# colopl/libpoporon

Hardware: AMD Instinct MI355X
Metric: RS(255,223) codewords/s (encode; decode @ t=16 errs) and GB/s vs HBM peak, 1/2/4/8 GPU (higher is better)
Workload: dtype u8; 1 GPU; RS(255,223) round trip: encode + decode with 16 errors per codeword, 1048576 codewords per GPU (BASELINE configs[1]+[2]); codewords_per_gpu=1048576, layout=255-byte codeword rows, stride 255, code=poporon_config_rs_default (8, 0x11D, fcr 1, prim 1, 32 roots)

## Files before the change

__graft_entry__.py:

```python
import os
import subprocess
import sys
import time

ROOT = os.path.dirname(os.path.abspath(__file__))


def build() -> None:
    subprocess.check_call(["make", "-j8", "-C", os.path.join(ROOT, "libpoporon_amd")])
    subprocess.check_call(["make", "-C", os.path.join(ROOT, "testutil")])
    subprocess.check_call(["make", "-C", os.path.join(ROOT, "tests", "c")])
    subprocess.check_call(["make", "-C", os.path.join(ROOT, "oracle")])
    if ROOT not in sys.path:
        sys.path.insert(0, ROOT)
    import libpoporon_amd

    libpoporon_amd.load_library()


def _errors(rng, bad, span, nerr, exclude=None):
    import numpy as np
    n = bad.shape[0]
    key = rng.random((n, span))
    if exclude is not None:
        np.put_along_axis(key, exclude.astype(np.int64), -1.0, axis=1)
    nmax = int(np.max(nerr))
    pos = np.argsort(-key, axis=1)[:, :nmax]
    mag = rng.integers(1, 256, (n, nmax), dtype=np.uint8)
    if not np.isscalar(nerr):
        mag[np.arange(nmax)[None, :] >= np.asarray(nerr)[:, None]] = 0
    r = np.arange(n)[:, None]
    bad[r, pos] ^= mag
    return pos


def smoke() -> None:
    if ROOT not in sys.path:
        sys.path.insert(0, ROOT)
    import numpy as np
    import torch

    import libpoporon_amd as P
    from oracle import Oracle

    assert torch.cuda.is_available(), "smoke() needs cuda:0"
    torch.cuda.set_device(0)
    t0 = time.perf_counter()
    prev_path = os.environ.get("POPORON_AMD_DECODE_PATH")
    os.environ["POPORON_AMD_DECODE_PATH"] = "split"
    try:
        rs = P.Poporon.default(device=0)
    finally:
        if prev_path is None:
            del os.environ["POPORON_AMD_DECODE_PATH"]
        else:
            os.environ["POPORON_AMD_DECODE_PATH"] = prev_path
    o = Oracle()
    th = min(16, os.cpu_count() or 1)
    rng = np.random.default_rng(0x5EED0001)
    n = 1 << 16
    K, NR = 223, 32
    s = torch.cuda.current_stream().cuda_stream

    data = rng.integers(0, 256, (n, K), dtype=np.uint8)
    cw = torch.zeros((n, 255), dtype=torch.uint8, device="cuda")
    cw[:, :K] = torch.from_numpy(data).cuda()
    rs.encode_batch_device(cw.data_ptr(), 255, cw.data_ptr() + K, 255, K, n, s)
    torch.cuda.synchronize()
    enc = cw.cpu().numpy()
    assert (enc[:, K:] == o.encode_batch(data, threads=th)).all(), "encode parity mismatch vs oracle"
    print(f"smoke encode: {n} messages, parity bit-exact vs oracle (rs_lfsr_k<ENCODE>)", flush=True)

    names = P.KERNEL_NAMES

    def decode(label, bad, expect, slots=None, cnt=None, kernels=""):
        d = torch.from_numpy(bad).cuda()
        ok = torch.zeros(n, dtype=torch.uint8, device="cuda")
        cor = torch.zeros(n, dtype=torch.uint8, device="cuda")
        kw = {}
        if slots is not None:
            sd = torch.from_numpy(np.ascontiguousarray(slots)).cuda()
            cd = torch.from_numpy(np.ascontiguousarray(cnt)).cuda()
            kw = dict(d_positions=sd.data_ptr(), positions_stride=slots.shape[1], d_counts=cd.data_ptr())
        rs.timing(True)
        rs.decode_batch_device(d.data_ptr(), 255, d.data_ptr() + K, 255, K, n, ok.data_ptr(), cor.data_ptr(),
                               stream=s, **kw)
        torch.cuda.synchronize()
        t = {k: rs.timing_read(k) for k in names}
        rs.timing(False)
        ran = {k for k, (ms, c) in t.items() if c}
        missing = [names[k] for k in expect if k not in ran]
        assert not missing, f"{label}: kernels that did not run: {missing}"
        assert P.KERNEL_CORRECT not in ran, f"{label}: the whole-batch general kernel ran instead of the split path"
        if slots is None:
            want = o.decode_batch(bad[:, :K], bad[:, K:], threads=th)
        else:
            want = o.decode_batch(bad[:, :K], bad[:, K:], slots.astype(np.uint32), cnt.astype(np.uint32), threads=th)
        out = d.cpu().numpy()
        gok, gcor = ok.cpu().numpy(), cor.cpu().numpy()
        assert (gok == want[0]).all(), f"{label}: ok differs at {np.nonzero(gok != want[0])[0][:8]}"
        assert (gcor == want[1]).all(), f"{label}: corrected_num differs at {np.nonzero(gcor != want[1])[0][:8]}"
        diff = np.nonzero((out[:, :K] != want[2]).any(1) | (out[:, K:] != want[3]).any(1))[0]
        assert diff.size == 0, f"{label}: decoded bytes differ at codewords {diff[:8]}"
        print(f"smoke {label}: {n} codewords bit-exact vs oracle (bytes, ok, corrected_num); ok {int(gok.sum())}, "
              f"corrected {int(gcor.sum())}; ran {kernels or ', '.join(names[k] for k in sorted(ran))}", flush=True)
        return gok, gcor, out

    bad = enc.copy()
    _errors(rng, bad, 255, 16)
    gok, gcor, out = decode("decode16", bad, (P.KERNEL_REMAINDER, P.KERNEL_BM, P.KERNEL_CHIEN, P.KERNEL_FORNEY,
                                              P.KERNEL_APPLY, P.KERNEL_LIST),
                            kernels="rs_lfsr_k<SYNDROME>, rs_bm_k, rs_chien_k, rs_forney_k, rs_apply_k<16>, "
                                    "rs_wave_k (list, empty)")
    assert gok.all() and (gcor == 16).all() and (out == enc).all()

    bad = enc.copy()
    slots = np.sort(np.argsort(rng.random((n, K)), axis=1)[:, :NR], axis=1).astype(np.uint8)
    bad[np.arange(n)[:, None], slots] ^= rng.integers(1, 256, (n, NR), dtype=np.uint8)
    cnt = np.full(n, NR, np.uint8)
    gok, gcor, out = decode("erasure32", bad, (P.KERNEL_REMAINDER, P.KERNEL_ERASURE, P.KERNEL_APPLY), slots, cnt,
                            kernels="rs_lfsr_k<SYNDROME>, rs_era_bp_k, rs_apply_k<32>")
    assert gok.all() and (gcor == NR).all() and (out == enc).all()

    bad = enc.copy()
    era = np.argsort(rng.random((n, K)), axis=1)[:, :16]
    slots = rng.integers(0, 255, (n, NR)).astype(np.uint8)
    slots[:, :16] = era
    bad[np.arange(n)[:, None], era] ^= rng.integers(1, 256, (n, 16), dtype=np.uint8)
    _errors(rng, bad, 255, 8, exclude=era)
    cnt = np.full(n, 16, np.uint8)
    decode("errata16e8", bad, (P.KERNEL_REMAINDER, P.KERNEL_ERASURE, P.KERNEL_BM, P.KERNEL_CHIEN, P.KERNEL_FORNEY,
                               P.KERNEL_APPLY, P.KERNEL_LIST), slots, cnt,
           kernels="rs_lfsr_k<SYNDROME>, rs_era_bp_k (hand-off), rs_ebm_k, rs_chien32_k, rs_forney32_k, "
                   "rs_wave_k (list), rs_apply_k<32>")

    bad = enc.copy()
    ne = np.minimum(rng.binomial(255, 0.045, n), 24)
    _errors(rng, bad, 255, ne)
    gok, _, _ = decode("mixed", bad, (P.KERNEL_REMAINDER, P.KERNEL_BM, P.KERNEL_CHIEN, P.KERNEL_FORNEY,
                                      P.KERNEL_APPLY, P.KERNEL_LIST),
                       kernels="rs_lfsr_k<SYNDROME>, rs_bm_k, rs_chien_k, rs_forney_k, rs_apply_k<16>, "
                               "rs_wave_k (list: L > 16 / deg != L, one wave per codeword)")
    assert (ne > 16).sum() > n // 50 and (gok == 0).sum() > 0

    for c in range(8):
        par = rs.encode(data[c])
        assert (par == enc[c, K:]).all(), "poporon_encode mismatch"
        b = enc[c].copy()
        _errors(rng, b[None, :], 255, 16 + (c & 1) * 2)
        got = rs.decode(b[:K], b[K:])
        want = o.decode(b[:K], b[K:])
        assert got[0] == want[0] and got[1] == want[1] and (got[2] == want[2]).all() and (got[3] == want[3]).all()
    print("smoke single calls: 8 x poporon_encode + poporon_decode (16 / 18 errors) bit-exact vs oracle "
          "(the single-call server rs_serve_k: enc1_body / dec1_body)", flush=True)
    print(f"smoke ok ({time.perf_counter() - t0:.1f} s)", flush=True)


if __name__ == "__main__":
    build()
    if len(sys.argv) > 1 and sys.argv[1] == "smoke":
        smoke()
```

libpoporon_amd/csrc/api.cpp:

```cpp
#include <hip/hip_runtime.h>

#include <algorithm>
#include <atomic>
#include <chrono>
#include <cstdarg>
#include <cstdio>
#include <cstdlib>
#include <cstring>
#include <mutex>
#include <new>
#include <string>
#include <thread>
#include <vector>

#include "poporon.h"
#include "poporon_amd.h"
#include "rs_device.h"
#include "rs_generic.h"
#include "bch_device.h"

#ifndef POPORON_BUILDTIME
#define POPORON_BUILDTIME 1
#endif
#define POPORON_VERSION_ID 20000000
// ... 68 lines not shown

struct GpuCtx {
    bool timing = false;
    std::vector<TimedLaunch> pending;
    std::vector<hipEvent_t> event_pool;
    double total_ms[NKERN] = {};
    uint64_t launches[NKERN] = {};
    bool ready = false;
    int device = -1;
    int num_cu = 256;
    hipStream_t stream = nullptr;
    RsDevTables *tab = nullptr;
    RsGenTables *gtab = nullptr;
    uint8_t *rem = nullptr;
    size_t rem_cap = 0;
    hipEvent_t rem_done = nullptr;
    hipStream_t rem_stream = nullptr;
    bool rem_pending = false;
    uint8_t *stage = nullptr;
    uint8_t *hstage = nullptr;
    uint8_t *zc = nullptr, *zc_dev = nullptr;
    uint32_t zc_seq = 0;
    hipStream_t sstream = nullptr;
    bool srv_on = false;
    uint32_t srv_id = 0;
    uint32_t srv_seq = 0;
    size_t stage_cap = 0;
    bool registered = false;
    bool batch_open = false;
    bool batch_ev_live = false;
    hipEvent_t batch_ev = nullptr;
    struct PipeSlot {
        hipStream_t stream = nullptr;
        hipEvent_t done = nullptr;
        uint8_t *host = nullptr;
        uint8_t *dev = nullptr;
        size_t cap = 0;
        bool busy = false;
        size_t c0 = 0, n = 0;
    } pipe[3];
};
#define PIPE_SLOTS 3

struct _poporon_t {
    poporon_fec_type_t fec_type;
    poporon_rs_t *rs;
    uint16_t primitive_inverse;
    poporon_erasure_t *erasure;
    uint16_t *ext_syndrome;
    size_t last_corrected;
    bool supported;
    bool fast;
    int decode_path;
    bool generic;
    bool lfsr_nr;
    bool nrsplit;
    int gen_path;
    RsDevTables host_tab;
    RsCorrParams corr;
    RsGenTables gen_tab;
    RsGenParams gen;
    poporon_gf_t *bgf;
    BchParams bch;
    bool bch_ok;
    GpuCtx gpu;
};


static inline uint8_t gf_mod(const poporon_gf_t *gf, uint16_t v)
{
    while (v >= gf->field_size) {
        v = (uint16_t)(v - gf->field_size);
        v = (uint16_t)((v >> gf->symbol_size) + (v & gf->field_size));
    }
    return (uint8_t)v;
}

EXPORT void poporon_gf_destroy(poporon_gf_t *gf)
{
    if (!gf)
        return;
    free(gf->log2exp);
    free(gf->exp2log);
    free(gf);
}

EXPORT poporon_gf_t *poporon_gf_create(uint8_t symbol_size, uint16_t generator_polynomial)
{
    if (symbol_size < 1 || symbol_size > 16)
        return nullptr;
    poporon_gf_t *gf = (poporon_gf_t *)calloc(1, sizeof(poporon_gf_t));
    if (!gf)
        return nullptr;
    gf->symbol_size = symbol_size;
    gf->field_size = (uint8_t)((1u << symbol_size) - 1u);
    gf->generator_polynomial = generator_polynomial;
    gf->log2exp = (uint16_t *)calloc((size_t)gf->field_size + 1, sizeof(uint16_t));
    gf->exp2log = (uint16_t *)calloc((size_t)gf->field_size + 1, sizeof(uint16_t));
    if (!gf->log2exp || !gf->exp2log) {
        poporon_gf_destroy(gf);
        return nullptr;
    }
    gf->exp2log[0] = gf->field_size;
    gf->log2exp[gf->field_size] = 0;
    uint16_t x = 1;
    for (uint8_t i = 0; i < gf->field_size; i++) {
// ... 236 lines not shown

    RsCorrParams &p = h->corr;
    memset(&p, 0, sizeof(p));
    p.fcr = rs->first_consecutive_root;
    p.prim = rs->primitive_element;
    p.iprim = h->primitive_inverse;
    p.vfast = ((uint64_t)(p.fcr + nr - 1) * p.prim * 254u) < 32768u;
    p.nr = nr;

    auto gmul = [&](uint32_t x, uint32_t logc) -> uint8_t {
        return x == 0 ? 0 : (uint8_t)gf->log2exp[(gf->exp2log[x] + logc) % 255];
    };
    for (uint32_t m = 0; m < RS_NR; m++) {
        for (uint32_t n = 0; n < 2; n++) {
            for (uint32_t v = 0; v < 16; v++) {
                uint8_t rowb[RS_NR];
                for (uint32_t i = 0; i < RS_NR; i++) {
                    if (m >= nr || i >= nr) {
                        rowb[i] = 0;
                        continue;
                    }
                    const uint64_t e = (uint64_t)(nr - 1 - m) * p.prim * (p.fcr + i);
                    rowb[i] = gmul(v << (4 * n), (uint32_t)(e % 255));
                }
                memcpy(&t.synt[((m * 2 + n) * 2 + 0) * 16 + v], rowb, 16);
                memcpy(&t.synt[((m * 2 + n) * 2 + 1) * 16 + v], rowb + 16, 16);
            }
        }
    }
    for (uint32_t j = 1; j <= 32; j++) {
        for (uint32_t e = 0; e < 256; e++) {
            uint8_t rowb[16];
            for (uint32_t b = 0; b < 16; b++)
                rowb[b] = e == 255 ? 0 : (uint8_t)gf->log2exp[(e + j * b) % 255];
            memcpy(&t.chien[(j - 1) * 256 + e], rowb, 16);
        }
    }
    uint32_t *gfa = reinterpret_cast<uint32_t *>(t.gfa);
    for (uint32_t x = 0; x < 512; x++)
        for (uint32_t r = 0; r < 32; r++) {
            const uint32_t la = x < 256u ? (x ? (uint32_t)t.log[x] * 128u + 4u * r + 1u : 128u * RS_Z0 + 4u * r) : 0u;
            gfa[x * 32 + r] = ((uint32_t)t.exp2[x] << 8) | (la << 16);
        }
    uint32_t *gfc = reinterpret_cast<uint32_t *>(t.gfc);
    for (uint32_t x = 0; x < 512; x++)
        for (uint32_t r = 0; r < 32; r++) {
            const uint32_t v = x & 255u;
            gfc[x * 32 + r] = ((uint32_t)t.exp2[x] << 8) | ((v ? (uint32_t)t.log[v] * 128u : 0xFFFFu) << 16);
        }
    const char *fv = getenv("POPORON_AMD_FORCE_VERIFY");
    p.force_verify = (fv && fv[0] == '1') ? 1u : 0u;
    const char *dp = getenv("POPORON_AMD_DECODE_PATH");
    h->decode_path = !dp ? 0 : !strcmp(dp, "split") ? 1 : !strcmp(dp, "single") ? 2 : !strcmp(dp, "wave") ? 3 : 0;
}

static bool params_generic(const poporon_t *h)
{
    const poporon_rs_t *rs = h->rs;
    const uint32_t m = rs->gf->symbol_size, nn = rs->gf->field_size;
    return m >= 2 && m <= 8 && rs->num_roots >= 1 && rs->num_roots < nn && rs->primitive_element != 0;
}

static void build_generic(poporon_t *h)
{
    const poporon_rs_t *rs = h->rs;
    const poporon_gf_t *gf = rs->gf;
    RsGenTables &t = h->gen_tab;
    const uint32_t nn = gf->field_size;
    memset(&t, 0, sizeof(t));
    for (uint32_t i = 0; i < 256; i++) {
        t.alog[i] = i <= nn ? (uint8_t)gf->log2exp[i] : 0;
        t.log[i] = i <= nn ? (uint8_t)gf->exp2log[i] : (uint8_t)nn;
    }
    for (uint32_t i = 0; i <= rs->num_roots; i++)
        t.gen[i] = (uint8_t)rs->generator_polynomial[i];
    for (uint32_t fb = 0; fb < 256; fb++) {
        const uint32_t v = fb & nn;
        for (uint32_t i = 0; i < rs->num_roots && v != 0; i++)
            t.lrow[fb * 256 + i] = (uint8_t)gf->log2exp[gf_mod(
                gf, (uint16_t)(gf->exp2log[v] + rs->generator_polynomial[rs->num_roots - 1 - i]))];
    }
    {
        const uint32_t nr = rs->num_roots;
        const uint16_t *g = rs->generator_polynomial;
        memset(t.encq, 0xff, sizeof(t.encq));
        std::vector<uint8_t> reg(nr, 0);
        for (uint32_t d = 0; d < nn - nr; d++) {
            const uint32_t fb = gf->exp2log[(d == 0 ? 1u : 0u) ^ reg[0]];
            if (fb != nn)
                for (uint32_t j = 1; j < nr; j++)
                    reg[j] ^= (uint8_t)gf->log2exp[gf_mod(gf, (uint16_t)(fb + g[nr - j]))];
            for (uint32_t j = 0; j + 1 < nr; j++)
                reg[j] = reg[j + 1];
            reg[nr - 1] = fb != nn ? (uint8_t)gf->log2exp[gf_mod(gf, (uint16_t)(fb + g[0]))] : 0;
            for (uint32_t j = 0; j < nr; j++)
                t.encq[d * 256 + j] = reg[j] ? (uint8_t)gf->exp2log[reg[j]] : (uint8_t)0xff;
        }
    }
    RsGenParams &p = h->gen;
    memset(&p, 0, sizeof(p));
    p.m = gf->symbol_size;
    p.nn = nn;
    p.magic = (uint32_t)((1ull << 32) / nn) + 1u;
    p.fcr = rs->first_consecutive_root;
    p.prim = rs->primitive_element;
    p.iprim = h->primitive_inverse;
// ... 708 lines not shown
        HIP_OK(rsk_encode1_nr(h->gpu.tab, d_data, d_par, (uint32_t)size, h->rs->num_roots, nullptr, 0u, s));
    } else if (h->lfsr_nr && !h->gen_path) {
        HIP_OK(rsk_encode_nr(h->gpu.tab, d_data, ds, d_par, ps, (uint32_t)size, count, h->rs->num_roots,
                             h->gpu.num_cu, s));
    } else if (h->rs->num_roots > RS_NR && !h->gen_path && count >= GEN_LFSR_MIN) {
        RsGenParams prm = h->gen;
        prm.size = (uint32_t)size;
        HIP_OK(rsg_lfsr_encode(h->gpu.gtab, &prm, d_data, ds, d_par, ps, count, h->gpu.num_cu, s));
    } else {
        RsGenParams prm = h->gen;
        prm.size = (uint32_t)size;
        if (gen_wave(h, count, true, size))
            HIP_OK(rsgw_encode(h->gpu.gtab, &prm, d_data, ds, d_par, ps, count, nullptr, 0u, h->gpu.num_cu, s));
        else
            HIP_OK(rsg_encode(h->gpu.gtab, &prm, d_data, ds, d_par, ps, count, h->gpu.num_cu, s));
    }
    t.done();
    return true;
}

#define SPLIT_MIN_COUNT 16384

static bool launch_split(poporon_t *h, const RsCorrParams &prm, const RsSplitWs &ws, uint8_t *d_data, size_t ds,
                         uint8_t *d_par, size_t ps, size_t size, size_t count, uint8_t *ok, uint8_t *corrected,
                         hipStream_t s, uint32_t npar = RS_NR, const uint16_t *ext = nullptr, size_t ext_stride = 0)
{
    GpuCtx &g = h->gpu;
    const bool nr = npar < RS_NR;
    {
        KernelTimer t(g, POPORON_AMD_KERNEL_REMAINDER, s);
        if (ext)
            HIP_OK(rsk_ext_syn(g.tab, ext, ext_stride, count, npar, ws.syn, ws.list, ws.nlist, s));
        else if (nr)
            HIP_OK(rsk_syndrome_reset_nr(g.tab, d_data, ds, d_par, ps, (uint32_t)size, count, ws.syn, ws.nlist, npar,
                                         g.num_cu, s));
        else
            HIP_OK(rsk_syndrome_reset(g.tab, d_data, ds, d_par, ps, (uint32_t)size, count, ws.syn, ws.nlist,
                                      g.num_cu, s));
        t.done();
    }
    {
        KernelTimer t(g, POPORON_AMD_KERNEL_BM, s);
        if (nr)
            HIP_OK(rsk_bm_nr(g.tab, &ws, count, npar, ok, corrected, g.num_cu, s));
        else
            HIP_OK(rsk_bm(g.tab, &ws, count, ok, corrected, g.num_cu, s));
        t.done();
    }
    {
        KernelTimer t(g, POPORON_AMD_KERNEL_CHIEN, s);
        HIP_OK(rsk_chien(g.tab, &prm, &ws, count, ok, corrected, g.num_cu, s));
        t.done();
    }
    {
        KernelTimer t(g, POPORON_AMD_KERNEL_FORNEY, s);
        HIP_OK(rsk_forney(g.tab, &prm, &ws, d_data, ds, d_par, ps, count, ok, corrected, g.num_cu, s));
        t.done();
    }
    {
        KernelTimer t(g, POPORON_AMD_KERNEL_APPLY, s);
        if (nr)
            HIP_OK(rsk_apply_nr(&prm, &ws, d_data, ds, d_par, ps, count, npar, s));
        else
            HIP_OK(rsk_apply(&prm, &ws, d_data, ds, d_par, ps, count, s));
        t.done();
    }
    {
        KernelTimer t(g, POPORON_AMD_KERNEL_LIST, s);
        if (nr) {
            RsGenParams gp = h->gen;
            gp.size = (uint32_t)size;
            gp.pad = prm.pad;
            if (h->gen_path == 1)
                HIP_OK(rsg_decode_list(g.gtab, &gp, d_data, ds, d_par, ps, count, ws.list, ws.nlist, ext, ext_stride,
                                       nullptr, 0, nullptr, ok, corrected, g.num_cu, s));
            else
                HIP_OK(rsgw_decode(g.gtab, &gp, d_data, ds, d_par, ps, count, ext, ext_stride, nullptr, nullptr, 0,
                                   nullptr, ok, corrected, ws.list, ws.nlist, nullptr, 0u, g.num_cu, s));
        } else {
            HIP_OK(rsk_wave(g.tab, &prm, d_data, ds, d_par, ps, count, ws.list, ws.nlist, ext ? nullptr : ws.syn, ext,
                            ext_stride, nullptr, nullptr, 0, nullptr, ok, corrected, g.num_cu, s));
        }
        t.done();
    }
    return true;
}

static bool launch_decode(poporon_t *h, uint8_t *d_data, size_t ds, uint8_t *d_par, size_t ps, size_t size,
                          size_t count, const uint16_t *ext_syn, size_t ext_stride, const uint8_t *pos8,
                          const uint32_t *pos32, size_t pos_stride, const uint8_t *cnt, uint8_t *ok,
                          uint8_t *corrected, hipStream_t s, uint8_t *rem = nullptr, size_t rem_cap = 0)
{
    if (h->fec_type == PPLN_FEC_BCH) {
        if (ext_syn || pos8 || pos32)
            return fail("BCH has no erasure or external-syndrome decode");
        KernelTimer t(h->gpu, POPORON_AMD_KERNEL_CORRECT, s);
        HIP_OK(bchk_decode(&h->bch, d_data, ds, d_par, ps, count, ok, corrected, h->gpu.num_cu, s));
        t.done();
        return true;
    }
    if (h->nrsplit && count == 1 && h->decode_path == 0) {
        RsCorrParams prm = h->corr;
        prm.size = (uint32_t)size;
        prm.pad = (int32_t)(h->rs->gf->field_size - h->rs->num_roots - size);
        KernelTimer t(h->gpu, POPORON_AMD_KERNEL_SINGLE, s);
        HIP_OK(rsk_decode1(h->gpu.tab, &prm, ext_syn ? 2u : (pos8 || pos32) ? 1u : 0u, d_data, d_par, pos8, pos32,
                           cnt, 1u, ext_syn, ok, corrected, nullptr, 0, s));
        t.done();
        return true;
    }
    if (h->nrsplit && !pos8 && !pos32 && h->corr.vfast && !h->corr.force_verify &&
        (h->decode_path == 1 || h->decode_path == 0)) {
        RsCorrParams prm = h->corr;
        prm.size = (uint32_t)size;
        prm.pad = (int32_t)(h->rs->gf->field_size - h->rs->num_roots - size);
        const bool shared = !rem;
        if (shared) {
            if (!ensure_rem(h, count) || !rem_acquire(h->gpu, s))
// ... 1172 lines not shown
```

libpoporon_amd/csrc/rs_device.h:

```cpp
#ifndef POPORON_AMD_RS_DEVICE_H
#define POPORON_AMD_RS_DEVICE_H

#include <stddef.h>
#include <stdint.h>

#include <hip/hip_ext.h>
#include <hip/hip_runtime.h>

struct RsLaunchTimer {
    hipEvent_t start, stop;
    int n;
};
extern thread_local RsLaunchTimer rs_launch_timer;
#define RS_LAUNCH(K, G, B, SH, S, ...)                                                                    \
    do {                                                                                                 \
        if (rs_launch_timer.stop)                                                                        \
            hipExtLaunchKernelGGL(K, G, B, SH, S, rs_launch_timer.n++ ? nullptr : rs_launch_timer.start, \
                                  rs_launch_timer.stop, 0u, __VA_ARGS__);                                \
        else                                                                                             \
            hipLaunchKernelGGL(K, G, B, SH, S, __VA_ARGS__);                                             \
    } while (0)

#define RS_NR 32
#define RS_A0 255u
// ... 96 lines not shown
#define ZC_REQ_SIZE(w) ((w) & 0xFFu)
#define ZC_YIELD 708
#define ZC_EXITED 768
#define GZ_DATA 1024
#define GZ_PAR 1280
#define GZ_POS 1536
#define GZ_CNT 2560
#define GZ_EXT 2576
#define GZ_OK 3088
#define GZ_COR 3089
#define ZC_BYTES 4096
#define RS_SRV_ENCODE 1u
#define RS_SRV_DECODE 2u
#define RS_SRV_STOP 3u

hipError_t rsk_wave(const RsDevTables *tab, const RsCorrParams *prm, uint8_t *data, size_t dstride, uint8_t *parity,
                    size_t pstride, size_t count, const uint32_t *list, const uint32_t *list_n, const uint8_t *syn,
                    const uint16_t *syn16, size_t syn16_stride, const uint8_t *pos8, const uint32_t *pos32,
                    size_t pos_stride, const uint8_t *cnt, uint8_t *ok, uint8_t *corrected, int num_cu,
                    hipStream_t stream);

hipError_t rsk_syn_log(const RsDevTables *tab, const uint8_t *syn, size_t count, uint16_t *out, size_t stride,
                       uint8_t *flag, hipStream_t stream);

hipError_t rsk_check(const RsDevTables *tab, const uint8_t *data, size_t dstride, const uint8_t *parity, size_t pstride,
                     uint32_t size, size_t count, uint8_t *flag, int num_cu, hipStream_t stream);
hipError_t rsk_ext_syn(const RsDevTables *tab, const uint16_t *ext, size_t ext_stride, size_t count, uint32_t npar,
                       uint8_t *syn, uint32_t *list, uint32_t *nlist, hipStream_t stream);
hipError_t rsk_syn_log_nr(const RsDevTables *tab, const uint8_t *syn, size_t count, uint16_t *out, size_t stride,
                          uint8_t *flag, uint32_t npar, hipStream_t stream);
hipError_t rsk_check_nr(const RsDevTables *tab, const uint8_t *data, size_t dstride, const uint8_t *parity,
                        size_t pstride, uint32_t size, size_t count, uint8_t *flag, uint32_t npar, int num_cu,
                        hipStream_t stream);

hipError_t rsk_correct(const RsDevTables *tab, const RsCorrParams *prm, uint8_t *data, size_t dstride, uint8_t *parity,
                       size_t pstride, size_t count, const uint8_t *syn, const uint16_t *syn16, size_t syn16_stride,
                       const uint8_t *pos8,
                       const uint32_t *pos32, size_t pos_stride, const uint8_t *cnt, uint8_t *ok, uint8_t *corrected,
                       int num_cu, hipStream_t stream);

hipError_t rsk_correct_list(const RsDevTables *tab, const RsCorrParams *prm, uint8_t *data, size_t dstride,
                            uint8_t *parity, size_t pstride, size_t count, const uint8_t *syn, const uint32_t *list,
                            const uint32_t *list_n, uint8_t *ok, uint8_t *corrected, int num_cu, hipStream_t stream);

hipError_t rsk_bm(const RsDevTables *tab, const RsSplitWs *ws, size_t count, uint8_t *ok, uint8_t *corrected,
                  int num_cu, hipStream_t stream);
hipError_t rsk_chien(const RsDevTables *tab, const RsCorrParams *prm, const RsSplitWs *ws, size_t count, uint8_t *ok,
                     uint8_t *corrected, int num_cu, hipStream_t stream);
hipError_t rsk_forney(const RsDevTables *tab, const RsCorrParams *prm, const RsSplitWs *ws, uint8_t *data,
                      size_t dstride, uint8_t *parity, size_t pstride, size_t count, uint8_t *ok, uint8_t *corrected,
                      int num_cu, hipStream_t stream);
hipError_t rsk_apply(const RsCorrParams *prm, const RsSplitWs *ws, uint8_t *data, size_t dstride, uint8_t *parity,
                     size_t pstride, size_t count, hipStream_t stream);

hipError_t rsk_syndrome_reset_nr(const RsDevTables *tab, const uint8_t *data, size_t dstride, const uint8_t *parity,
                                 size_t pstride, uint32_t size, size_t count, uint8_t *syn, uint32_t *reset,
                                 uint32_t npar, int num_cu, hipStream_t stream);
hipError_t rsk_bm_nr(const RsDevTables *tab, const RsSplitWs *ws, size_t count, uint32_t npar, uint8_t *ok,
                     uint8_t *corrected, int num_cu, hipStream_t stream);
hipError_t rsk_apply_nr(const RsCorrParams *prm, const RsSplitWs *ws, uint8_t *data, size_t dstride, uint8_t *parity,
                        size_t pstride, size_t count, uint32_t npar, hipStream_t stream);
hipError_t rsk_ebm_nr(const RsDevTables *tab, const RsCorrParams *prm, const RsSplitWs *ws, const uint8_t *pos8,
                      size_t pos_stride, const uint8_t *cnt, size_t count, uint8_t *ok, uint8_t *corrected,
                      uint32_t npar, int num_cu, hipStream_t stream);
hipError_t rsk_forney32_nr(const RsDevTables *tab, const RsCorrParams *prm, const RsSplitWs *ws, const uint8_t *pos8,
                           size_t pos_stride, size_t count, uint8_t *ok, uint8_t *corrected, uint32_t npar,
                           int num_cu, hipStream_t stream);
hipError_t rsk_apply_era_nr(const RsCorrParams *prm, const uint8_t *meta, const uint8_t *rec, uint8_t *data,
                            size_t dstride, uint8_t *parity, size_t pstride, size_t count, uint32_t npar,
                            hipStream_t stream);

hipError_t rsk_correct_era_rec(const RsDevTables *tab, const RsCorrParams *prm, size_t count, const uint8_t *syn,
                               const uint8_t *pos8, const uint32_t *pos32, size_t pos_stride, const uint8_t *cnt,
                               uint8_t *ok, uint8_t *corrected, uint8_t *rec, uint8_t *meta, int num_cu,
                               hipStream_t stream);
hipError_t rsk_era(const RsDevTables *tab, const RsCorrParams *prm, const RsSplitWs *ws, const uint8_t *pos8,
                   size_t pos_stride, const uint8_t *cnt, size_t count, uint8_t *ok, uint8_t *corrected, uint32_t pend,
                   int num_cu, hipStream_t stream);
hipError_t rsk_correct_era_list(const RsDevTables *tab, const RsCorrParams *prm, size_t count, const uint8_t *syn,
                                const uint8_t *pos8, size_t pos_stride, const uint8_t *cnt, uint8_t *ok,
                                uint8_t *corrected, uint8_t *rec, uint8_t *meta, const uint32_t *list,
                                const uint32_t *list_n, int num_cu, hipStream_t stream);
hipError_t rsk_apply_era(const RsCorrParams *prm, const uint8_t *meta, const uint8_t *rec, uint8_t *data,
                         size_t dstride, uint8_t *parity, size_t pstride, size_t count, hipStream_t stream);

hipError_t rsk_ebm(const RsDevTables *tab, const RsCorrParams *prm, const RsSplitWs *ws, const uint8_t *pos8,
                   size_t pos_stride, const uint8_t *cnt, size_t count, uint8_t *ok, uint8_t *corrected,
                   uint32_t only_pend, int num_cu, hipStream_t stream);
hipError_t rsk_chien32(const RsDevTables *tab, const RsCorrParams *prm, const RsSplitWs *ws, size_t count, uint8_t *ok,
                       uint8_t *corrected, uint32_t only_pend, int num_cu, hipStream_t stream);
hipError_t rsk_forney32(const RsDevTables *tab, const RsCorrParams *prm, const RsSplitWs *ws, const uint8_t *pos8,
                        size_t pos_stride, size_t count, uint8_t *ok, uint8_t *corrected, uint32_t only_pend,
                        int num_cu, hipStream_t stream);

#ifdef __cplusplus
}
#endif

#endif
```

libpoporon_amd/csrc/rs_fast.hip:

```cpp
#include <hip/hip_runtime.h>

#include <type_traits>

#include "rs_device.h"
#include "rs_gfa.h"
#include "rs_lane.h"

#define FWG 1024
#define NL 17
#define BWG 512
#define BM_WAVES 4

#define FAST_ROUNDS 8
static int fast_grid(size_t count, int num_cu)
{
    const size_t need = (count + FWG - 1) / FWG;
    const size_t g = FAST_ROUNDS * 2u * (size_t)(num_cu > 0 ? num_cu : 256);
    return (int)(need < g ? (need ? need : 1) : g);
}


template <bool NRG>
__global__ __launch_bounds__(BWG, BM_WAVES) void rs_bm_k(const RsDevTables *__restrict__ T, const uint8_t *__restrict__ syn,
                                                   size_t count, uint8_t *__restrict__ lamo, uint8_t *__restrict__ omo,
// ... 629 lines not shown
        return;
    const uint32_t lim = size + npar;
    if (wire && base + 64u <= count) {
        const uint4 *src = reinterpret_cast<const uint4 *>(data + base * 255u);
        uint4 *dst = reinterpret_cast<uint4 *>(data + base * 255u);
        uint4 *im = img[w];
#pragma unroll
        for (uint32_t k = 0; k < 16; ++k) {
            const uint32_t c = lane + 64u * k;
            if (c < ABLK) {
                const lds_u32x4_t v = __builtin_nontemporal_load(reinterpret_cast<const lds_u32x4_t *>(src + c));
                im[c] = make_uint4(v.x, v.y, v.z, v.w);
            }
        }
        __builtin_amdgcn_fence(__ATOMIC_RELEASE, "wavefront");
        __builtin_amdgcn_wave_barrier();
        __builtin_amdgcn_fence(__ATOMIC_ACQUIRE, "wavefront");
        uint32_t *imw = reinterpret_cast<uint32_t *>(im);
#pragma unroll
        for (int n = 0; n < NC; ++n) {
            const uint32_t mg = (mw[n >> 2] >> (8 * (n & 3))) & 0xffu;
            const uint32_t p = (pw[n >> 2] >> (8 * (n & 3))) & 0xffu;
            if (mg && p < lim) {
                const uint32_t b = lane * 255u + p;
                atomicXor(imw + (b >> 2), mg << (8u * (b & 3u)));
            }
        }
        __builtin_amdgcn_fence(__ATOMIC_RELEASE, "wavefront");
        __builtin_amdgcn_wave_barrier();
        __builtin_amdgcn_fence(__ATOMIC_ACQUIRE, "wavefront");
#pragma unroll
        for (uint32_t k = 0; k < 16; ++k) {
            const uint32_t c = lane + 64u * k;
            if (c < ABLK) {
                const uint4 v = im[c];
                __builtin_nontemporal_store(lds_u32x4_t{v.x, v.y, v.z, v.w}, reinterpret_cast<lds_u32x4_t *>(dst + c));
            }
        }
    } else if (fast) {
        uint8_t *cdata = data + cw * dstride, *cpar = parity + cw * pstride;
#pragma unroll
        for (int n = 0; n < NC; ++n) {
            const uint32_t mg = (mw[n >> 2] >> (8 * (n & 3))) & 0xffu;
            const uint32_t p = (pw[n >> 2] >> (8 * (n & 3))) & 0xffu;
            if (mg && p < lim) {
                uint8_t *d = p < size ? cdata + p : cpar + (p - size);
                *d = (uint8_t)(*d ^ mg);
            }
        }
    }
}


extern "C" hipError_t rsk_bm(const RsDevTables *tab, const RsSplitWs *ws, size_t count, uint8_t *ok,
                             uint8_t *corrected, int num_cu, hipStream_t stream)
{
    if (count == 0)
        return hipSuccess;
    const size_t need = (count + BWG - 1) / BWG,
                 res = FAST_ROUNDS * (size_t)(num_cu > 0 ? num_cu : 256) * (BM_WAVES * 256 / BWG);
    RS_LAUNCH(rs_bm_k<false>, dim3((uint32_t)(need < res ? need : res)), dim3(BWG), 0, stream, tab, ws->syn, count,
              ws->lam, ws->om, ws->meta, ws->list, ws->nlist, ok, corrected, (uint32_t)RS_NR);
    return hipGetLastError();
}

extern "C" hipError_t rsk_bm_nr(const RsDevTables *tab, const RsSplitWs *ws, size_t count, uint32_t npar, uint8_t *ok,
                                uint8_t *corrected, int num_cu, hipStream_t stream)
{
    if (count == 0)
        return hipSuccess;
    const size_t need = (count + BWG - 1) / BWG,
                 res = FAST_ROUNDS * (size_t)(num_cu > 0 ? num_cu : 256) * (BM_WAVES * 256 / BWG);
    RS_LAUNCH(rs_bm_k<true>, dim3((uint32_t)(need < res ? need : res)), dim3(BWG), 0, stream, tab, ws->syn, count,
              ws->lam, ws->om, ws->meta, ws->list, ws->nlist, ok, corrected, npar);
    return hipGetLastError();
}

extern "C" hipError_t rsk_chien(const RsDevTables *tab, const RsCorrParams *prm, const RsSplitWs *ws, size_t count,
                                uint8_t *ok, uint8_t *corrected, int num_cu, hipStream_t stream)
{
    if (count == 0)
        return hipSuccess;
    RS_LAUNCH(rs_chien_k, dim3(fast_grid(count, num_cu)), dim3(FWG), 0, stream, tab, *prm, count, ws->lam,
                       ws->meta, ws->roots, ok, corrected);
    return hipGetLastError();
}

extern "C" hipError_t rsk_forney(const RsDevTables *tab, const RsCorrParams *prm, const RsSplitWs *ws, uint8_t *data,
                                 size_t dstride, uint8_t *parity, size_t pstride, size_t count, uint8_t *ok,
                                 uint8_t *corrected, int num_cu, hipStream_t stream)
{
    if (count == 0)
        return hipSuccess;
    const size_t need = (count + F2WG - 1) / F2WG, cap = FAST_ROUNDS * 2u * (size_t)(num_cu > 0 ? num_cu : 256);
    const dim3 grid((uint32_t)(need < cap ? need : cap));
    if (prm->fcr == 1u && prm->iprim == 1u)
        RS_LAUNCH(rs_forney_k<true>, grid, dim3(F2WG), 0, stream, tab, *prm, data, dstride, parity, pstride, count,
                  ws->lam, ws->om, ws->roots, ws->meta, ok, corrected);
    else
        RS_LAUNCH(rs_forney_k<false>, grid, dim3(F2WG), 0, stream, tab, *prm, data, dstride, parity, pstride, count,
                  ws->lam, ws->om, ws->roots, ws->meta, ok, corrected);
    return hipGetLastError();
}

template <int NC>
static hipError_t apply_launch(const RsCorrParams *prm, const uint8_t *meta, const uint8_t *rec, uint8_t *data,
                               size_t dstride, uint8_t *parity, size_t pstride, size_t count, hipStream_t stream,
                               uint32_t npar = RS_NR)
{
    if (count == 0)
        return hipSuccess;
    const uint32_t wire = prm->size + npar == 255u && dstride == 255u && pstride == 255u &&
                          parity == data + prm->size && (reinterpret_cast<uintptr_t>(data) & 15u) == 0u;
    const size_t waves = (count + 63) / 64;
    RS_LAUNCH(rs_apply_k<NC>, dim3((uint32_t)((waves + AWG / 64 - 1) / (AWG / 64))), dim3(AWG), 0, stream,
                       meta, rec, data, dstride, parity, pstride, prm->size, count, wire, npar);
    return hipGetLastError();
}

extern "C" hipError_t rsk_apply(const RsCorrParams *prm, const RsSplitWs *ws, uint8_t *data, size_t dstride,
                                uint8_t *parity, size_t pstride, size_t count, hipStream_t stream)
{
    return apply_launch<16>(prm, ws->meta, ws->roots, data, dstride, parity, pstride, count, stream);
}

extern "C" hipError_t rsk_apply_nr(const RsCorrParams *prm, const RsSplitWs *ws, uint8_t *data, size_t dstride,
                                   uint8_t *parity, size_t pstride, size_t count, uint32_t npar, hipStream_t stream)
{
    return apply_launch<16>(prm, ws->meta, ws->roots, data, dstride, parity, pstride, count, stream, npar);
}

extern "C" hipError_t rsk_apply_era_nr(const RsCorrParams *prm, const uint8_t *meta, const uint8_t *rec, uint8_t *data,
                                       size_t dstride, uint8_t *parity, size_t pstride, size_t count, uint32_t npar,
                                       hipStream_t stream)
{
    return apply_launch<32>(prm, meta, rec, data, dstride, parity, pstride, count, stream, npar);
}

extern "C" hipError_t rsk_apply_era(const RsCorrParams *prm, const uint8_t *meta, const uint8_t *rec, uint8_t *data,
                                    size_t dstride, uint8_t *parity, size_t pstride, size_t count, hipStream_t stream)
{
    return apply_launch<32>(prm, meta, rec, data, dstride, parity, pstride, count, stream);
}

extern "C" hipError_t rsk_era(const RsDevTables *tab, const RsCorrParams *prm, const RsSplitWs *ws, const uint8_t *pos8,
                              size_t pos_stride, const uint8_t *cnt, size_t count, uint8_t *ok, uint8_t *corrected,
                              uint32_t pend, int num_cu, hipStream_t stream)
{
    if (count == 0)
        return hipSuccess;
    const size_t need = (count + BPWG - 1) / BPWG,
                 res = (size_t)(num_cu > 0 ? num_cu : 256) * (BP_WAVES * 256 / BPWG);
    RS_LAUNCH(rs_era_bp_k, dim3((uint32_t)(need < res ? need : res)), dim3(BPWG), 0, stream, tab, *prm, ws->syn,
              pos8, pos_stride, cnt, count, ws->ext, ws->meta, ws->list, ws->nlist, ok, corrected, pend);
    return hipGetLastError();
}
```

Before: 2.024 billion codewords/s.

## Fuse Forney magnitude computation with in-place error application in one kernel

Adds rs_forney_apply_k, which computes error positions and magnitudes per lane and applies them to the codeword rows in the same kernel. For wire-layout batches it stages each 64-row tile through LDS, with part of the row loads issued before the Forney arithmetic so they can overlap it. This removes one launch and the global round-trip of the per-codeword correction records between the old Forney and apply kernels. The fused tail becomes the default unless the split decode path is forced by environment. The cost is one large-LDS, 1024-thread block per CU, which can lower occupancy relative to the separate kernels.

```diff
diff --git a/__graft_entry__.py b/__graft_entry__.py
--- a/__graft_entry__.py
+++ b/__graft_entry__.py
@@ -46,15 +46,17 @@
     assert torch.cuda.is_available(), "smoke() needs cuda:0"
     torch.cuda.set_device(0)
     t0 = time.perf_counter()
-    prev_path = os.environ.get("POPORON_AMD_DECODE_PATH")
-    os.environ["POPORON_AMD_DECODE_PATH"] = "split"
+    want_env = {"POPORON_AMD_DECODE_PATH": "split", "POPORON_AMD_DECODE_TAIL": "fused"}
+    prev_env = {k: os.environ.get(k) for k in want_env}
+    os.environ.update(want_env)
     try:
         rs = P.Poporon.default(device=0)
     finally:
-        if prev_path is None:
-            del os.environ["POPORON_AMD_DECODE_PATH"]
-        else:
-            os.environ["POPORON_AMD_DECODE_PATH"] = prev_path
+        for k, v in prev_env.items():
+            if v is None:
+                del os.environ[k]
+            else:
+                os.environ[k] = v
     o = Oracle()
     th = min(16, os.cpu_count() or 1)
     rng = np.random.default_rng(0x5EED0001)
@@ -108,9 +110,9 @@
 
     bad = enc.copy()
     _errors(rng, bad, 255, 16)
-    gok, gcor, out = decode("decode16", bad, (P.KERNEL_REMAINDER, P.KERNEL_BM, P.KERNEL_CHIEN, P.KERNEL_FORNEY,
-                                              P.KERNEL_APPLY, P.KERNEL_LIST),
-                            kernels="rs_lfsr_k<SYNDROME>, rs_bm_k, rs_chien_k, rs_forney_k, rs_apply_k<16>, "
+    gok, gcor, out = decode("decode16", bad, (P.KERNEL_REMAINDER, P.KERNEL_BM, P.KERNEL_CHIEN, P.KERNEL_APPLY,
+                                              P.KERNEL_LIST),
+                            kernels="rs_lfsr_k<SYNDROME>, rs_bm_k, rs_chien_k, rs_forney_apply_k, "
                                     "rs_wave_k (list, empty)")
     assert gok.all() and (gcor == 16).all() and (out == enc).all()
 
@@ -137,9 +139,8 @@
     bad = enc.copy()
     ne = np.minimum(rng.binomial(255, 0.045, n), 24)
     _errors(rng, bad, 255, ne)
-    gok, _, _ = decode("mixed", bad, (P.KERNEL_REMAINDER, P.KERNEL_BM, P.KERNEL_CHIEN, P.KERNEL_FORNEY,
-                                      P.KERNEL_APPLY, P.KERNEL_LIST),
-                       kernels="rs_lfsr_k<SYNDROME>, rs_bm_k, rs_chien_k, rs_forney_k, rs_apply_k<16>, "
+    gok, _, _ = decode("mixed", bad, (P.KERNEL_REMAINDER, P.KERNEL_BM, P.KERNEL_CHIEN, P.KERNEL_APPLY, P.KERNEL_LIST),
+                       kernels="rs_lfsr_k<SYNDROME>, rs_bm_k, rs_chien_k, rs_forney_apply_k, "
                                "rs_wave_k (list: L > 16 / deg != L, one wave per codeword)")
     assert (ne > 16).sum() > n // 50 and (gok == 0).sum() > 0
 
diff --git a/libpoporon_amd/csrc/api.cpp b/libpoporon_amd/csrc/api.cpp
--- a/libpoporon_amd/csrc/api.cpp
+++ b/libpoporon_amd/csrc/api.cpp
@@ -144,6 +144,7 @@
     bool supported;
     bool fast;
     int decode_path;
+    int decode_tail;
     bool generic;
     bool lfsr_nr;
     bool nrsplit;
@@ -486,6 +487,8 @@
     p.force_verify = (fv && fv[0] == '1') ? 1u : 0u;
     const char *dp = getenv("POPORON_AMD_DECODE_PATH");
     h->decode_path = !dp ? 0 : !strcmp(dp, "split") ? 1 : !strcmp(dp, "single") ? 2 : !strcmp(dp, "wave") ? 3 : 0;
+    const char *dt = getenv("POPORON_AMD_DECODE_TAIL");
+    h->decode_tail = dt && !strcmp(dt, "split") ? 1 : dt && !strcmp(dt, "fused") ? 0 : h->decode_path == 1 ? 1 : 0;
 }
 
 static bool params_generic(const poporon_t *h)
@@ -1300,18 +1303,24 @@
         HIP_OK(rsk_chien(g.tab, &prm, &ws, count, ok, corrected, g.num_cu, s));
         t.done();
     }
-    {
-        KernelTimer t(g, POPORON_AMD_KERNEL_FORNEY, s);
-        HIP_OK(rsk_forney(g.tab, &prm, &ws, d_data, ds, d_par, ps, count, ok, corrected, g.num_cu, s));
+    if (h->decode_tail == 0) {
+        KernelTimer t(g, POPORON_AMD_KERNEL_APPLY, s);
+        HIP_OK(rsk_forney_apply(g.tab, &prm, &ws, d_data, ds, d_par, ps, count, npar, ok, corrected, g.num_cu, s));
         t.done();
-    }
-    {
-        KernelTimer t(g, POPORON_AMD_KERNEL_APPLY, s);
-        if (nr)
-            HIP_OK(rsk_apply_nr(&prm, &ws, d_data, ds, d_par, ps, count, npar, s));
-        else
-            HIP_OK(rsk_apply(&prm, &ws, d_data, ds, d_par, ps, count, s));
-        t.done();
+    } else {
+        {
+            KernelTimer t(g, POPORON_AMD_KERNEL_FORNEY, s);
+            HIP_OK(rsk_forney(g.tab, &prm, &ws, d_data, ds, d_par, ps, count, ok, corrected, g.num_cu, s));
+            t.done();
+        }
+        {
+            KernelTimer t(g, POPORON_AMD_KERNEL_APPLY, s);
+            if (nr)
+                HIP_OK(rsk_apply_nr(&prm, &ws, d_data, ds, d_par, ps, count, npar, s));
+            else
+                HIP_OK(rsk_apply(&prm, &ws, d_data, ds, d_par, ps, count, s));
+            t.done();
+        }
     }
     {
         KernelTimer t(g, POPORON_AMD_KERNEL_LIST, s);
diff --git a/libpoporon_amd/csrc/rs_device.h b/libpoporon_amd/csrc/rs_device.h
--- a/libpoporon_amd/csrc/rs_device.h
+++ b/libpoporon_amd/csrc/rs_device.h
@@ -172,6 +172,9 @@
                       int num_cu, hipStream_t stream);
 hipError_t rsk_apply(const RsCorrParams *prm, const RsSplitWs *ws, uint8_t *data, size_t dstride, uint8_t *parity,
                      size_t pstride, size_t count, hipStream_t stream);
+hipError_t rsk_forney_apply(const RsDevTables *tab, const RsCorrParams *prm, const RsSplitWs *ws, uint8_t *data,
+                            size_t dstride, uint8_t *parity, size_t pstride, size_t count, uint32_t npar, uint8_t *ok,
+                            uint8_t *corrected, int num_cu, hipStream_t stream);
 
 hipError_t rsk_syndrome_reset_nr(const RsDevTables *tab, const uint8_t *data, size_t dstride, const uint8_t *parity,
                                  size_t pstride, uint32_t size, size_t count, uint8_t *syn, uint32_t *reset,
diff --git a/libpoporon_amd/csrc/rs_fast.hip b/libpoporon_amd/csrc/rs_fast.hip
--- a/libpoporon_amd/csrc/rs_fast.hip
+++ b/libpoporon_amd/csrc/rs_fast.hip
@@ -705,6 +705,197 @@
 }
 
 
+#define FAWG 1024
+#define FAQ 255u
+#ifndef FA_PRE
+#define FA_PRE 2
+#endif
+
+template <bool P11>
+__device__ __forceinline__ uint32_t forney_lane(const GfA gf, const uint32_t fcr, const uint32_t iprim,
+                                                const int32_t pad, uint32_t deg, const uint4 o4, const uint4 l4,
+                                                const uint32_t (&rl)[4], uint32_t (&posp)[4], uint32_t (&magp)[4])
+{
+    constexpr bool fcr1 = P11, iprim1 = P11;
+    constexpr int R = FORNEY_R;
+    const uint32_t mp = 255u * 128u + gf.pofs;
+    const uint32_t ow[4] = {o4.x, o4.y, o4.z, o4.w}, lw[4] = {l4.x, l4.y, l4.z, l4.w};
+    const uint32_t dtop = deg ? (deg - 1u) & ~1u : 0u;
+    uint32_t opu[16], lod[8];
+#pragma unroll
+    for (int m = 0; m < 16; ++m)
+        opu[m] = gf.afrom((ow[m >> 2] >> (8 * (m & 3))) & 0xffu);
+#pragma unroll
+    for (int h = 0; h < 8; ++h)
+        lod[h] = (uint32_t)(2 * h) <= dtop ? gf.afrom((lw[(2 * h) >> 2] >> (8 * ((2 * h) & 3))) & 0xffu) : gf.az();
+    const uint32_t degmax = wave_max(deg);
+    uint32_t fixed = 0;
+#pragma unroll
+    for (int k = 0; k < 4; ++k)
+        posp[k] = magp[k] = 0;
+#pragma unroll
+    for (int n0 = 0; n0 < 16; n0 += R) {
+        if ((uint32_t)n0 >= degmax)
+            continue;
+        uint32_t ir[R], si[R], s[R], num[R], den[R], nh[R], dh[R];
+#pragma unroll
+        for (int t = 0; t < R; ++t) {
+            ir[t] = root_point((rl[(n0 + t) >> 2] >> (8 * ((n0 + t) & 3))) & 0xffu);
+            si[t] = 128u * (ir[t] == 255u ? 0u : ir[t]);
+            s[t] = num[t] = den[t] = nh[t] = dh[t] = 0;
+        }
+#pragma unroll
+        for (int b = 0; b < 8; ++b) {
+#pragma unroll
+            for (int t = 0; t < R; ++t) {
+                num[t] ^= gf.expa(opu[b] + s[t]);
+                nh[t] ^= gf.expa(opu[b + 8] + s[t]);
+                if ((b & 1) == 0) {
+                    den[t] ^= gf.expa(lod[b >> 1] + s[t]);
+                    dh[t] ^= gf.expa(lod[(b >> 1) + 4] + s[t]);
+                }
+                s[t] = addmod7(s[t], si[t]);
+            }
+            if (b & 1) {
+#pragma unroll
+                for (int t = 0; t < R; ++t)
+                    asm volatile("" : "+v"(num[t]), "+v"(den[t]), "+v"(nh[t]), "+v"(dh[t]));
+                __builtin_amdgcn_sched_barrier(0);
+            }
+        }
+#pragma unroll
+        for (int t = 0; t < R; ++t) {
+            num[t] ^= gf.expa(gf.loga(nh[t]) + s[t]);
+            den[t] ^= gf.expa(gf.loga(dh[t]) + s[t]);
+            uint32_t mag;
+            if constexpr (fcr1) {
+                mag = gf.expa(gf.loga(num[t]) - gf.loga(den[t]) + mp);
+            } else {
+                const uint32_t ln2 = mod255((uint32_t)((int32_t)ir[t] * ((int32_t)fcr - 1) + (int32_t)RS_NN));
+                const uint32_t lden = gf.plog(gf.loga(den[t]));
+                mag = gf.exp(red(gf.plog(gf.loga(num[t])) + ln2 + RS_NN - lden));
+            }
+            const bool z = (uint32_t)(n0 + t) < deg && num[t] != 0u;
+            fixed += z ? 1u : 0u;
+            const uint32_t k = iprim1 ? ir[t] - 1u : (ir[t] * iprim + 254u) % 255u;
+            const uint32_t p = (uint32_t)((int32_t)k - pad);
+            posp[(n0 + t) >> 2] |= (p & 0xffu) << (8 * ((n0 + t) & 3));
+            magp[(n0 + t) >> 2] |= (z ? mag : 0u) << (8 * ((n0 + t) & 3));
+        }
+        __builtin_amdgcn_sched_barrier(0);
+    }
+    return fixed;
+}
+
+template <bool P11>
+__global__ __launch_bounds__(FAWG, FAWG / 256) void rs_forney_apply_k(
+    const RsDevTables *__restrict__ T, RsCorrParams P, uint8_t *data, size_t dstride, uint8_t *parity, size_t pstride,
+    size_t count, const uint8_t *__restrict__ lam, const uint8_t *__restrict__ om, const uint8_t *__restrict__ roots,
+    const uint8_t *__restrict__ meta, uint8_t *__restrict__ ok, uint8_t *__restrict__ corrected, uint32_t wire,
+    uint32_t npar)
+{
+    __shared__ uint32_t lgf[512 * 32];
+    __shared__ uint4 stage[FAWG / 64][256];
+    fill_gfa<FAWG>(lgf, T);
+    __syncthreads();
+    const GfA gf{lds_addr(lgf) + 4u * (threadIdx.x & 31u) + 1u};
+    const uint32_t lane = threadIdx.x & 63u;
+    uint4 *st = stage[threadIdx.x >> 6];
+    const uint32_t lim = P.size + npar;
+    const size_t nb = (count + FAWG - 1) / FAWG;
+
+    for (size_t b = blockIdx.x; b < nb; b += gridDim.x) {
+        const size_t wbase = (nb - 1u - b) * FAWG + (threadIdx.x & ~63u);
+        const size_t cw = wbase + lane;
+        const bool valid = cw < count;
+        const uint32_t mt = valid ? meta[cw] : 0u;
+        const bool fast = (mt >> 5) == RS_ST_FAST;
+        if (__ballot(fast) == 0ull)
+            continue;
+        const uint32_t deg = fast ? (mt & 31u) : 0u;
+        uint4 o4 = make_uint4(0xFFFFFFFFu, 0xFFFFFFFFu, 0xFFFFFFFFu, 0xFFFFFFFFu), l4 = o4;
+        uint32_t rl[4] = {0, 0, 0, 0};
+        if (fast) {
+            o4 = reinterpret_cast<const uint4 *>(om)[cw];
+            l4 = reinterpret_cast<const uint4 *>(lam)[cw];
+            const uint4 ra = reinterpret_cast<const uint4 *>(roots)[2 * cw];
+            rl[0] = ra.x, rl[1] = ra.y, rl[2] = ra.z, rl[3] = ra.w;
+        }
+        __builtin_amdgcn_sched_barrier(0);
+        const bool block = wire && wbase + 64u <= count;
+        lds_u32x4_t *rows = reinterpret_cast<lds_u32x4_t *>(data + wbase * 255u);
+        const uint32_t c3 = min(lane + 192u, FAQ - 1u);
+        const lds_u32x4_t *pre = block ? rows : reinterpret_cast<const lds_u32x4_t *>(T->gfa);
+        lds_u32x4_t v[4][4];
+#pragma unroll
+        for (int q = 0; q < FA_PRE; ++q)
+#pragma unroll
+            for (uint32_t k = 0; k < 4; ++k)
+                v[q][k] = __builtin_nontemporal_load(pre + FAQ * q + (k < 3 ? lane + 64u * k : c3));
+        __builtin_amdgcn_sched_barrier(0);
+        uint32_t posp[4], magp[4];
+        const uint32_t fixed = forney_lane<P11>(gf, P.fcr, P.iprim, P.pad, deg, o4, l4, rl, posp, magp);
+        if (fast) {
+            ok[cw] = 1;
+            if (corrected)
+                corrected[cw] = (uint8_t)fixed;
+        }
+        if (block) {
+#pragma unroll
+            for (int q = FA_PRE; q < 4; ++q)
+#pragma unroll
+                for (uint32_t k = 0; k < 4; ++k)
+                    v[q][k] = __builtin_nontemporal_load(rows + FAQ * q + (k < 3 ? lane + 64u * k : c3));
+            uint32_t *stw = reinterpret_cast<uint32_t *>(st);
+#pragma unroll
+            for (int q = 0; q < 4; ++q) {
+#pragma unroll
+                for (uint32_t k = 0; k < 4; ++k)
+                    if (lane + 64u * k < FAQ)
+                        st[lane + 64u * k] = make_uint4(v[q][k].x, v[q][k].y, v[q][k].z, v[q][k].w);
+                __builtin_amdgcn_fence(__ATOMIC_RELEASE, "wavefront");
+                __builtin_amdgcn_wave_barrier();
+                __builtin_amdgcn_fence(__ATOMIC_ACQUIRE, "wavefront");
+                if ((lane >> 4) == (uint32_t)q) {
+#pragma unroll
+                    for (int n = 0; n < 16; ++n) {
+                        const uint32_t mg = (magp[n >> 2] >> (8 * (n & 3))) & 0xffu;
+                        const uint32_t p = (posp[n >> 2] >> (8 * (n & 3))) & 0xffu;
+                        if (mg && p < lim) {
+                            const uint32_t a = (lane & 15u) * 255u + p;
+                            atomicXor(stw + (a >> 2), mg << (8u * (a & 3u)));
+                        }
+                    }
+                }
+                __builtin_amdgcn_fence(__ATOMIC_RELEASE, "wavefront");
+                __builtin_amdgcn_wave_barrier();
+                __builtin_amdgcn_fence(__ATOMIC_ACQUIRE, "wavefront");
+#pragma unroll
+                for (uint32_t k = 0; k < 4; ++k)
+                    if (lane + 64u * k < FAQ) {
+                        const uint4 r = st[lane + 64u * k];
+                        __builtin_nontemporal_store(lds_u32x4_t{r.x, r.y, r.z, r.w}, rows + FAQ * q + lane + 64u * k);
+                    }
+                __builtin_amdgcn_fence(__ATOMIC_RELEASE, "wavefront");
+                __builtin_amdgcn_wave_barrier();
+                __builtin_amdgcn_fence(__ATOMIC_ACQUIRE, "wavefront");
+            }
+        } else if (fast) {
+            uint8_t *cdata = data + cw * dstride, *cpar = parity + cw * pstride;
+#pragma unroll
+            for (int n = 0; n < 16; ++n) {
+                const uint32_t mg = (magp[n >> 2] >> (8 * (n & 3))) & 0xffu;
+                const uint32_t p = (posp[n >> 2] >> (8 * (n & 3))) & 0xffu;
+                if (mg && p < lim) {
+                    uint8_t *d = p < P.size ? cdata + p : cpar + (p - P.size);
+                    *d = (uint8_t)(*d ^ mg);
+                }
+            }
+        }
+    }
+}
+
+
 extern "C" hipError_t rsk_bm(const RsDevTables *tab, const RsSplitWs *ws, size_t count, uint8_t *ok,
                              uint8_t *corrected, int num_cu, hipStream_t stream)
 {
@@ -756,6 +947,25 @@
     return hipGetLastError();
 }
 
+extern "C" hipError_t rsk_forney_apply(const RsDevTables *tab, const RsCorrParams *prm, const RsSplitWs *ws,
+                                       uint8_t *data, size_t dstride, uint8_t *parity, size_t pstride, size_t count,
+                                       uint32_t npar, uint8_t *ok, uint8_t *corrected, int num_cu, hipStream_t stream)
+{
+    if (count == 0)
+        return hipSuccess;
+    const uint32_t wire = prm->size + npar == 255u && dstride == 255u && pstride == 255u &&
+                          parity == data + prm->size && (reinterpret_cast<uintptr_t>(data) & 15u) == 0u;
+    const size_t need = (count + FAWG - 1) / FAWG, cap = (size_t)(num_cu > 0 ? num_cu : 256);
+    const dim3 grid((uint32_t)(need < cap ? need : cap));
+    if (prm->fcr == 1u && prm->iprim == 1u)
+        RS_LAUNCH(rs_forney_apply_k<true>, grid, dim3(FAWG), 0, stream, tab, *prm, data, dstride, parity, pstride,
+                  count, ws->lam, ws->om, ws->roots, ws->meta, ok, corrected, wire, npar);
+    else
+        RS_LAUNCH(rs_forney_apply_k<false>, grid, dim3(FAWG), 0, stream, tab, *prm, data, dstride, parity, pstride,
+                  count, ws->lam, ws->om, ws->roots, ws->meta, ok, corrected, wire, npar);
+    return hipGetLastError();
+}
+
 template <int NC>
 static hipError_t apply_launch(const RsCorrParams *prm, const uint8_t *meta, const uint8_t *rec, uint8_t *data,
                                size_t dstride, uint8_t *parity, size_t pstride, size_t count, hipStream_t stream,
```

Result: faster. 2.102 billion codewords/s, median of 6 (+3.9%).
